# YufengJin/BundleSDF

Hardware: AMD Instinct MI355X
Metric: NeRF training rays/sec + ms/iter, 64-frame pool, 2048 rays/frame (higher is better)
Workload: dtype fp16 table+MLP (MFMA) / fp32 accumulate+Adam (amp)

## Files before the change

bundlesdf_amd/csrc/field_step.hip:

```cpp
#include <algorithm>
#include <cstdlib>
#include <cstring>
#include <array>
#include <type_traits>
#include <vector>

#include "nof_device.h"
#include "ray_trace.h"
#include "mlp_lds.h"

#pragma clang fp contract(off)

#ifndef NOF_ABLATE
#define NOF_ABLATE 0
#endif
#define ABL(bits) (NOF_ABLATE && (a.ablate & (bits)))
#define ABL_HOST(d, bits) (NOF_ABLATE && ((d)->ablate & (bits)))
#define ABL_SKIPQ(q) ((q) < 2 ? (1 << (23 + (q))) : (1 << (27 + (q))))

namespace nof {

typedef _Float16 h8v __attribute__((ext_vector_type(8)));
typedef float f16v __attribute__((ext_vector_type(16)));

// ... 346 lines not shown

__device__ __forceinline__ void corner_rows(const LevelInfo &li, const uint32_t pg[3], uint32_t rows[8]) {
    const uint32_t rs = li.res + 1;
    if (level_dense(rs, li.hs)) {
        const uint32_t base = dense_base_v(li.off, pg, rs), rs2 = rs * rs;
#pragma unroll
        for (int idx = 0; idx < 8; ++idx)
            rows[idx] = base + (idx & 1) + ((idx >> 1) & 1 ? rs : 0u) + ((idx >> 2) & 1 ? rs2 : 0u);
    } else {
#pragma unroll
        for (int idx = 0; idx < 8; ++idx) {
            uint32_t pl[3];
#pragma unroll
            for (int d = 0; d < 3; ++d) pl[d] = pg[d] + ((idx >> d) & 1);
            rows[idx] = li.off + grid_row<3>(0, false, li.hs, li.res, pl);
        }
    }
}

template <typename TT, bool PAIRED = false>
__device__ __forceinline__ void gather_level(const FieldArgs &a, const LevelInfo &li, const float x01[3], float pos[3],
                                             float e[8][2], uint32_t rows[8]) {
    const TT *tab = reinterpret_cast<const TT *>(a.table);
    uint32_t pg[3];
#pragma unroll
    for (int d = 0; d < 3; ++d) {
        pos[d] = __builtin_fmaf(x01[d], li.scale, 0.5f);
        pg[d] = (uint32_t)floorf(pos[d]);
        pos[d] -= (float)pg[d];
    }
    corner_rows(li, pg, rows);
    const uint32_t rs = li.res + 1;
    if (PAIRED && level_dense(rs, li.hs)) {
#pragma unroll
        for (int idx = 0; idx < 8; idx += 2) {
            const TT *p = tab + (size_t)rows[idx] * 2;
            if constexpr (sizeof(TT) == 4) {
                typedef float f4a __attribute__((ext_vector_type(4), aligned(8)));
                const f4a v = *reinterpret_cast<const f4a *>(p);
                e[idx][0] = v.x; e[idx][1] = v.y; e[idx + 1][0] = v.z; e[idx + 1][1] = v.w;
            } else {
                uint2 v;
                __builtin_memcpy(&v, p, 8);
                const __half2 h0 = __builtin_bit_cast(__half2, v.x), h1 = __builtin_bit_cast(__half2, v.y);
                e[idx][0] = __low2float(h0); e[idx][1] = __high2float(h0);
                e[idx + 1][0] = __low2float(h1); e[idx + 1][1] = __high2float(h1);
            }
        }
    } else {
#pragma unroll
        for (int idx = 0; idx < 8; ++idx) {
            const TT *p = tab + (size_t)rows[idx] * 2;
            if constexpr (sizeof(TT) == 4) {
                const float2 v = *reinterpret_cast<const float2 *>(p);
                e[idx][0] = v.x; e[idx][1] = v.y;
            } else {
                const __half2 v = *reinterpret_cast<const __half2 *>(p);
                e[idx][0] = __low2float(v); e[idx][1] = __high2float(v);
            }
        }
    }
}

template <typename TT>
__device__ __forceinline__ void encode_level(const FieldArgs &a, const LevelInfo &li, const float x01[3], float f[2]) {
    float pos[3], e[8][2];
    uint32_t rows[8];
    gather_level<TT, true>(a, li, x01, pos, e, rows);
    f[0] = 0.f; f[1] = 0.f;
#pragma unroll
    for (int idx = 0; idx < 8; ++idx) {
        float w = 1.f;
#pragma unroll
        for (int d = 0; d < 3; ++d) w *= ((idx >> d) & 1) ? pos[d] : 1 - pos[d];
        f[0] = __builtin_fmaf(w, e[idx][0], f[0]);
        f[1] = __builtin_fmaf(w, e[idx][1], f[1]);
    }
}

template <int CTRL> __device__ __forceinline__ int dpp_i(int v) {
    return __builtin_amdgcn_update_dpp(0, v, CTRL, 0xf, 0xf, true);
}
#define DPP_ROW_SHL(n) (0x100 + (n))
#define DPP_ROW_SHR(n) (0x110 + (n))

constexpr uint32_t SLOT_EMPTY = 0xffffffffu;

__device__ __forceinline__ uint32_t lds_cas(uint32_t *p, uint32_t key) {
    uint32_t e = SLOT_EMPTY;
    __hip_atomic_compare_exchange_strong(p, &e, key, __ATOMIC_RELAXED, __ATOMIC_RELAXED, __HIP_MEMORY_SCOPE_WORKGROUP);
    return e;
}

template <bool F16V> __device__ __forceinline__ uint32_t *slot_key(uint32_t *keys, uint32_t s) {
    return keys + (F16V ? 2 * s : s);
}
__device__ __forceinline__ void lds_add_h2(void *vals, uint32_t s, uint32_t packed) {
    __builtin_amdgcn_ds_atomic_fadd_v2f16(
        (__attribute__((address_space(3))) h2v *)(reinterpret_cast<uint32_t *>(vals) + 2 * s),
        __builtin_bit_cast(h2v, packed));
}
template <bool F16V>
__device__ __forceinline__ void lds_add(void *vals, uint32_t s, float v0, float v1) {
    if constexpr (F16V) {
        lds_add_h2(vals, s, __builtin_bit_cast(uint32_t, h2v{(_Float16)v0, (_Float16)v1}));
    } else {
        float *f = reinterpret_cast<float *>(vals) + 2 * s;
        __hip_atomic_fetch_add(f, v0, __ATOMIC_RELAXED, __HIP_MEMORY_SCOPE_WORKGROUP);
        __hip_atomic_fetch_add(f + 1, v1, __ATOMIC_RELAXED, __HIP_MEMORY_SCOPE_WORKGROUP);
    }
}

template <bool F16V>
__device__ __forceinline__ bool lds_probe(uint32_t *keys, void *vals, uint32_t mask, uint32_t key, float v0, float v1,
                                          float *g32, __half *g16) {
    uint32_t s = key;
#pragma unroll 1
    for (int p = 1; p < 16; ++p) {
        s = (s + 1) & mask;
        const uint32_t old = lds_cas(slot_key<F16V>(keys, s), key);
        if (old == SLOT_EMPTY || old == key) {
            lds_add<F16V>(vals, s, v0, v1);
            return true;
        }
    }
    if (g16) atomic_add_h2(g16 + (size_t)key * 2, v0, v1);
    else { atomic_add_f32(g32 + (size_t)key * 2, v0); atomic_add_f32(g32 + (size_t)key * 2 + 1, v1); }
    return false;
}

__device__ __forceinline__ void gather_level_t16(const FieldArgs &a, const LevelInfo &li, h2v g01, float t[8],
                                                 const uint32_t rows[8]) {
    const __half *tab = reinterpret_cast<const __half *>(a.table);
    const uint32_t rs = li.res + 1;
    if (level_dense(rs, li.hs)) {
#pragma unroll
        for (int idx = 0; idx < 8; idx += 2) {
            uint2 v;
            __builtin_memcpy(&v, tab + (size_t)rows[idx] * 2, 8);
            t[idx] = __builtin_amdgcn_fdot2(__builtin_bit_cast(h2v, v.x), g01, 0.f, false);
            t[idx + 1] = __builtin_amdgcn_fdot2(__builtin_bit_cast(h2v, v.y), g01, 0.f, false);
        }
    } else {
#pragma unroll
        for (int idx = 0; idx < 8; ++idx) {
            const uint32_t v = *reinterpret_cast<const uint32_t *>(tab + (size_t)rows[idx] * 2);
            t[idx] = __builtin_amdgcn_fdot2(__builtin_bit_cast(h2v, v), g01, 0.f, false);
        }
    }
}

template <typename TT, bool F16V>
__device__ __forceinline__ void backward_level(const FieldArgs &a, const LevelInfo &li, bool member, bool active,
                                               uint32_t part, const float x01[3], float g0, float g1, h2v g01,
                                               float gx[3], int lane, uint32_t *keys, void *vals, uint32_t mask,
                                               float *g32, __half *g16, int &n_direct) {
    float pos[3];
    uint32_t pg[3], crow[8];
#pragma unroll
    for (int d = 0; d < 3; ++d) {
        pos[d] = __builtin_fmaf(x01[d], li.scale, 0.5f);
        pg[d] = (uint32_t)pos[d];
        pos[d] = __builtin_amdgcn_fractf(pos[d]);
    }
    corner_rows(li, pg, crow);
    if (active && !a.no_dx) {
        float t[8];
        if constexpr (sizeof(TT) == 2) {
            gather_level_t16(a, li, g01, t, crow);
        } else {
            float e[8][2], pos_unused[3];
            uint32_t rows_unused[8];
            gather_level<TT, true>(a, li, x01, pos_unused, e, rows_unused);
#pragma unroll
            for (int k = 0; k < 8; ++k) t[k] = __builtin_fmaf(g1, e[k][1], g0 * e[k][0]);
        }
        float dx[4], ax[4];
#pragma unroll
        for (int j = 0; j < 4; ++j) {
            dx[j] = t[2 * j + 1] - t[2 * j];
            ax[j] = __builtin_fmaf(pos[0], dx[j], t[2 * j]);
        }
        float dy[2], by[2], ux[2];
#pragma unroll
        for (int z = 0; z < 2; ++z) {
            dy[z] = ax[2 * z + 1] - ax[2 * z];
            by[z] = __builtin_fmaf(pos[1], dy[z], ax[2 * z]);
            ux[z] = __builtin_fmaf(pos[1], dx[2 * z + 1] - dx[2 * z], dx[2 * z]);
        }
        gx[0] = __builtin_fmaf(li.scale, __builtin_fmaf(pos[2], ux[1] - ux[0], ux[0]), gx[0]);
        gx[1] = __builtin_fmaf(li.scale, __builtin_fmaf(pos[2], dy[1] - dy[0], dy[0]), gx[1]);
        gx[2] = __builtin_fmaf(li.scale, by[1] - by[0], gx[2]);
    }
    if ABL(1) return;
    const int key = member ? (int)((1u + (pg[0] | (pg[1] << 10) | (pg[2] << 20))) | (part << 31))
                           : (0x40000000 + lane + 1);
    const bool tail = member && (dpp_i<0x130>(key) != key);
    if (ABL(1 << 27)) {
        n_direct += tail ? 1 : 0;
    }
    const bool s1 = dpp_i<DPP_ROW_SHR(1)>(key) == key, s2 = dpp_i<DPP_ROW_SHR(2)>(key) == key;
    const bool s4 = dpp_i<DPP_ROW_SHR(4)>(key) == key, s8 = dpp_i<DPP_ROW_SHR(8)>(key) == key;
    const bool sb15 = __builtin_amdgcn_update_dpp(0, key, 0x142, 0xa, 0xf, false) == key;
    const bool sb31 = __builtin_amdgcn_update_dpp(0, key, 0x143, 0xc, 0xf, false) == key;
    const bool any1 = __any(s1), any2 = __any(s2);
    const bool any4 = __any(s4), any8 = __any(s8);
    const bool anyb15 = __any(sb15), anyb31 = __any(sb31);
    const float h0 = active ? g0 : 0.f, h1 = active ? g1 : 0.f;
    float wxy[4];
#pragma unroll
    for (int j = 0; j < 4; ++j) wxy[j] = ((j & 1) ? pos[0] : 1 - pos[0]) * ((j & 2) ? pos[1] : 1 - pos[1]);
    const float wz0[2] = {(1 - pos[2]) * h0, pos[2] * h0}, wz1[2] = {(1 - pos[2]) * h1, pos[2] * h1};
    float v0[8], v1[8];
#pragma unroll
    for (int idx = 0; idx < 8; ++idx) {
        v0[idx] = wxy[idx & 3] * wz0[idx >> 2];
        v1[idx] = wxy[idx & 3] * wz1[idx >> 2];
    }
    uint32_t pk[8];
    const bool pscan = F16V && !ABL(4096);
    if (pscan) {
#pragma unroll
        for (int idx = 0; idx < 8; ++idx) pk[idx] = __builtin_bit_cast(uint32_t, h2v{(_Float16)v0[idx], (_Float16)v1[idx]});
#define PFMAC_DPP(I, CTRL) "v_pk_fmac_f16_dpp %" #I ", %" #I ", %8 " CTRL "\n"
#define PSCAN_STEP(SK, CTRL)                                                                                      \
        if (any##SK) {                                                                                            \
            const uint32_t m = s##SK ? 0x3C003C00u : 0u;                                                          \
            asm("s_nop 1\n" PFMAC_DPP(0, CTRL) PFMAC_DPP(1, CTRL) PFMAC_DPP(2, CTRL) PFMAC_DPP(3, CTRL)          \
                PFMAC_DPP(4, CTRL) PFMAC_DPP(5, CTRL) PFMAC_DPP(6, CTRL) PFMAC_DPP(7, CTRL)                      \
                : "+v"(pk[0]), "+v"(pk[1]), "+v"(pk[2]), "+v"(pk[3]), "+v"(pk[4]), "+v"(pk[5]), "+v"(pk[6]),     \
                  "+v"(pk[7])                                                                                     \
                : "v"(m));                                                                                        \
        }
        PSCAN_STEP(1, "row_shr:1 row_mask:0xf bank_mask:0xf bound_ctrl:1")
        PSCAN_STEP(2, "row_shr:2 row_mask:0xf bank_mask:0xf bound_ctrl:1")
        PSCAN_STEP(4, "row_shr:4 row_mask:0xf bank_mask:0xf bound_ctrl:1")
        PSCAN_STEP(8, "row_shr:8 row_mask:0xf bank_mask:0xf bound_ctrl:1")
        PSCAN_STEP(b15, "row_bcast:15 row_mask:0xa bank_mask:0xf")
        PSCAN_STEP(b31, "row_bcast:31 row_mask:0xc bank_mask:0xf")
#undef PFMAC_DPP
#undef PSCAN_STEP
    }
#define FMAC_DPP(I, CTRL) "v_fmac_f32_dpp %" #I ", %" #I ", %16 " CTRL "\n"
#define SCAN_STEP(SK, CTRL)                                                                                       \
    if (!pscan && any##SK) {                                                                                      \
        const float m = s##SK ? 1.f : 0.f;                                                                        \
        asm("s_nop 1\n" FMAC_DPP(0, CTRL) FMAC_DPP(1, CTRL) FMAC_DPP(2, CTRL) FMAC_DPP(3, CTRL)                  \
            FMAC_DPP(4, CTRL) FMAC_DPP(5, CTRL) FMAC_DPP(6, CTRL) FMAC_DPP(7, CTRL) FMAC_DPP(8, CTRL)            \
            FMAC_DPP(9, CTRL) FMAC_DPP(10, CTRL) FMAC_DPP(11, CTRL) FMAC_DPP(12, CTRL) FMAC_DPP(13, CTRL)        \
            FMAC_DPP(14, CTRL) FMAC_DPP(15, CTRL)                                                                \
            : "+v"(v0[0]), "+v"(v0[1]), "+v"(v0[2]), "+v"(v0[3]), "+v"(v0[4]), "+v"(v0[5]), "+v"(v0[6]),         \
              "+v"(v0[7]), "+v"(v1[0]), "+v"(v1[1]), "+v"(v1[2]), "+v"(v1[3]), "+v"(v1[4]), "+v"(v1[5]),         \
              "+v"(v1[6]), "+v"(v1[7])                                                                            \
            : "v"(m));                                                                                            \
    }
    SCAN_STEP(1, "row_shr:1 row_mask:0xf bank_mask:0xf bound_ctrl:1")
    SCAN_STEP(2, "row_shr:2 row_mask:0xf bank_mask:0xf bound_ctrl:1")
    SCAN_STEP(4, "row_shr:4 row_mask:0xf bank_mask:0xf bound_ctrl:1")
    SCAN_STEP(8, "row_shr:8 row_mask:0xf bank_mask:0xf bound_ctrl:1")
    SCAN_STEP(b15, "row_bcast:15 row_mask:0xa bank_mask:0xf")
    SCAN_STEP(b31, "row_bcast:31 row_mask:0xc bank_mask:0xf")
#undef FMAC_DPP
#undef SCAN_STEP
    if (!tail) return;
    if (ABL(1 << 26)) {
        n_direct += (v0[0] + v1[7] == 12345.f || (pscan && pk[3] == 12345u)) ? 1 : 0;
        return;
    }
    if constexpr (F16V) {
        if (!pscan) {
#pragma unroll
            for (int idx = 0; idx < 8; ++idx)
                pk[idx] = __builtin_bit_cast(uint32_t, h2v{(_Float16)v0[idx], (_Float16)v1[idx]});
        }
    }
    uint32_t old[8];
#pragma unroll
    for (int idx = 0; idx < 8; ++idx) old[idx] = lds_cas(slot_key<F16V>(keys, crow[idx] & mask), crow[idx]);
    bool all_ok = true;
#pragma unroll
    for (int idx = 0; idx < 8; ++idx) {
        const bool ok = old[idx] == SLOT_EMPTY || old[idx] == crow[idx];
        all_ok = all_ok && ok;
        if constexpr (F16V) {
            lds_add_h2(vals, crow[idx] & mask, ok ? pk[idx] : 0u);
        } else {
            lds_add<F16V>(vals, crow[idx] & mask, ok ? v0[idx] : 0.f, ok ? v1[idx] : 0.f);
        }
    }
    if (__builtin_expect(__any(!all_ok), 0)) {
#pragma unroll
        for (int idx = 0; idx < 8; ++idx)
            if (!(old[idx] == SLOT_EMPTY || old[idx] == crow[idx])) {
                float u0 = v0[idx], u1 = v1[idx];
                if constexpr (F16V) {
                    const h2v q = __builtin_bit_cast(h2v, pk[idx]);
                    u0 = (float)q[0];
                    u1 = (float)q[1];
                }
                n_direct += lds_probe<F16V>(keys, vals, mask, crow[idx], u0, u1, g32, g16) ? 0 : 1;
            }
    }
}

template <bool F16V, int NJ>
__device__ __forceinline__ int flush_group(uint32_t *keys, void *vals, uint32_t s0, int lane, float *g32, __half *g16,
                                           bool no_hbm) {
    uint32_t k[NJ];
    uint32_t vb[NJ];
    float va[NJ], vc[NJ];
#pragma unroll
    for (int j = 0; j < NJ; ++j) {
        const uint32_t sl = s0 + 64 * j + lane;
        if constexpr (F16V) {
            const uint2 kv = reinterpret_cast<const uint2 *>(keys)[sl];
            k[j] = kv.x;
            vb[j] = kv.y;
        } else {
            k[j] = keys[sl];
            const float2 v = reinterpret_cast<float2 *>(vals)[sl];
            va[j] = v.x; vc[j] = v.y;
        }
    }
#pragma unroll
    for (int j = 0; j < NJ; ++j) {
        const uint32_t sl = s0 + 64 * j + lane;
        if constexpr (F16V) {
            reinterpret_cast<uint2 *>(keys)[sl] = make_uint2(0xffffffffu, 0u);
        } else {
            keys[sl] = 0xffffffffu;
            reinterpret_cast<float2 *>(vals)[sl] = make_float2(0.f, 0.f);
        }
    }
    int n = 0;
#pragma unroll
    for (int j = 0; j < NJ; ++j) {
        n += (int)__popcll(__ballot(k[j] != 0xffffffffu));
        if (k[j] != 0xffffffffu && !no_hbm) {
            if constexpr (F16V) {
                typedef _Float16 h2v __attribute__((ext_vector_type(2)));
                __builtin_amdgcn_global_atomic_fadd_v2f16((__attribute__((address_space(1))) h2v *)(g16 + (size_t)k[j] * 2),
                                                          __builtin_bit_cast(h2v, vb[j]));
            } else if (g16) {
                atomic_add_h2(g16 + (size_t)k[j] * 2, va[j], vc[j]);
            } else {
                atomic_add_f32(g32 + (size_t)k[j] * 2, va[j]);
                atomic_add_f32(g32 + (size_t)k[j] * 2 + 1, vc[j]);
            }
        }
// ... 802 lines not shown
            reinterpret_cast<float2 *>(a.tile_aux + slot * TILE_AUX + min(lane, 2))[1] = d;
        }
        float s0, s1, s2, sf;
        half_sums(h == 0 ? rc[0] : rc[1], s0, s1);
        half_sums(h == 0 ? rc[2] : lf, s2, sf);
        reinterpret_cast<float4 *>(a.rrec + slot * TREC)[2] = make_float4(s0, s1, s2, sf);
        cur = nxt;
        nxt = nn;
    }
}

__global__ __launch_bounds__(256) void k_ray_final(FieldArgs a_) {
    const FieldArgs a = step_args(a_);
    const int r = blockIdx.x * blockDim.x + threadIdx.x;
    const int lane = threadIdx.x & 63, wave = threadIdx.x >> 6;
    float v[10];
#pragma unroll
    for (int k = 0; k < 10; ++k) v[k] = 0.f;
    if (r < a.R) {
        const int ntiles = a.S / 32;
        float wtot = 0.f, nvalid = 0.f, lfs = 0.f, lem = 0.f, lsdf = 0.f, lfsr = 0.f;
        float racc[3] = {0.f, 0.f, 0.f};
        int csig = 0, ccol = 0, crcol = 0, crsig = 0;
#pragma unroll 4
        for (int t = 0; t < ntiles; ++t) {
            const size_t slot = (size_t)r * ntiles + t;
            const float4 *q = reinterpret_cast<const float4 *>(a.rrec + slot * TREC);
            const float4 q0 = q[0], q1 = q[1], q2 = q[2];
            const uint8_t fl = a.tile_bwd[slot];
            wtot += q0.x; nvalid += q0.y; lfs += q0.z; lem += q0.w; lsdf += q1.x;
            const int cnt = __float_as_int(q1.y);
            csig += cnt & TC_SIG; ccol += (cnt >> 1) & 1; crcol += (cnt >> 2) & 1; crsig += (cnt >> 3) & 1;
            if (fl == 1 || fl == 3) {
                racc[0] += q2.x; racc[1] += q2.y; racc[2] += q2.z; lfsr += q2.w;
            }
        }
        const float *cx = a.rctx + (size_t)r * RCTX;
        const float tgt[3] = {cx[3], cx[4], cx[5]};
        const int frame = __float_as_int(cx[23]), rtype = __float_as_int(cx[24]);
        const bool vray = nvalid > 0.f && rtype == 0;
        const float rw = vray ? (frame == 0 ? a.ffw : 1.f) : 0.f;
        float drgb[3], lr = 0.f, rgb[3];
#pragma unroll
        for (int cc = 0; cc < 3; ++cc) {
            rgb[cc] = racc[cc] / (wtot + 1e-10f);
            const float e = rgb[cc] - tgt[cc];
            drgb[cc] = a.rgb_w * 2.f * e * rw * a.inv_3R;
            lr += e * e * rw;
        }
        v[0] = a.rgb_w * lr * a.inv_3R;
        v[1] = lfs * rw;
        v[2] = lem * rw;
        v[3] = lsdf * rw;
        v[4] = nvalid;
        v[5] = lfsr * rw;
        v[6] = (float)csig; v[7] = (float)ccol; v[8] = (float)crcol; v[9] = (float)crsig;
        if (a.dbg_rgb) {
            a.dbg_rgb[r * 3] = rgb[0]; a.dbg_rgb[r * 3 + 1] = rgb[1]; a.dbg_rgb[r * 3 + 2] = rgb[2];
        }
        float4 *ra = reinterpret_cast<float4 *>(a.ray_aux + (size_t)r * RAY_AUX);
        ra[0] = make_float4(drgb[0], drgb[1], drgb[2], wtot);
        ra[1] = make_float4(rw, 0.f, 0.f, 0.f);
        float4 *rg = reinterpret_cast<float4 *>(a.ray_grad + (size_t)r * 12);
        rg[0] = make_float4(0.f, 0.f, 0.f, 0.f);
        rg[1] = make_float4(0.f, 0.f, 0.f, 0.f);
        rg[2] = make_float4(0.f, 0.f, 0.f, 0.f);
    }
    __shared__ float s_v[4][10];
#pragma unroll
    for (int k = 0; k < 10; ++k) {
        const float t = wave_sum(v[k]);
        if (lane == 0) s_v[wave][k] = t;
    }
    __syncthreads();
    if (threadIdx.x < 10) {
        const int k = threadIdx.x;
        const float t = s_v[0][k] + s_v[1][k] + s_v[2][k] + s_v[3][k];
        constexpr int slot[10] = {0, 1, 2, 3, 4, 10, 6, 7, 8, 9};
        if (t != 0.f && (k != 5 || a.fs_rgb_w > 0.f)) atomic_add_f32(loss_row(a, (int)blockIdx.x) + slot[k], t);
    }
}

constexpr int ENCODE_GROUP_SMALL = 2;

constexpr int COMPACT_PER_BLOCK = 4096;
__global__ __launch_bounds__(256) void k_compact(const uint8_t *__restrict__ flags, int n, int *__restrict__ list,
                                                 int *__restrict__ count, int per_block, int *__restrict__ clist) {
    __shared__ int s_wave[3][4];
    __shared__ int s_base[3];
    const int lane = threadIdx.x & 63, wave = threadIdx.x >> 6;
    const int fpt = per_block >> 8;
    const int b0 = blockIdx.x * per_block + threadIdx.x * fpt;
    uint8_t fl[16];
    if (fpt == 16 && b0 + 16 <= n) {
        const uint4 v = *reinterpret_cast<const uint4 *>(flags + b0);
        const uint32_t w[4] = {v.x, v.y, v.z, v.w};
#pragma unroll
        for (int k = 0; k < 16; ++k) fl[k] = (uint8_t)(w[k >> 2] >> (8 * (k & 3)));
    } else {
#pragma unroll
        for (int k = 0; k < 16; ++k) fl[k] = (k < fpt && b0 + k < n) ? flags[b0 + k] : 0;
    }
    int mine[3] = {0, 0, 0};
#pragma unroll
    for (int k = 0; k < 16; ++k) {
        mine[0] += fl[k] == 1;
        mine[1] += fl[k] == 2;
        mine[2] += (fl[k] == 1 || fl[k] == 3);
    }
    int pm[3] = {mine[0], mine[1], mine[2]};
#pragma unroll
    for (int o = 1; o < 64; o <<= 1) {
#pragma unroll
        for (int q = 0; q < 3; ++q) {
            const int u = __shfl_up(pm[q], o, 64);
            if (lane >= o) pm[q] += u;
        }
    }
    if (lane == 63) {
#pragma unroll
        for (int q = 0; q < 3; ++q) s_wave[q][wave] = pm[q];
    }
    __syncthreads();
    if (threadIdx.x < 3) {
        const int q = threadIdx.x;
        const int tot = s_wave[q][0] + s_wave[q][1] + s_wave[q][2] + s_wave[q][3];
        int *cnt = count + (q == 0 ? 0 : (q == 1 ? 2 : 1));
        s_base[q] = (tot && (q < 2 || clist)) ? atomicAdd(cnt, tot) : 0;
    }
    __syncthreads();
    int off[3];
#pragma unroll
    for (int q = 0; q < 3; ++q) {
        off[q] = s_base[q] + pm[q] - mine[q];
        for (int w = 0; w < wave; ++w) off[q] += s_wave[q][w];
    }
#pragma unroll
    for (int k = 0; k < 16; ++k) {
        const int i = b0 + k;
        if (fl[k] == 1) list[off[0]++] = i << 5;
        if (fl[k] == 2) list[n - 1 - off[1]++] = (i << 5) | (int)0x80000000;
        if (clist && (fl[k] == 1 || fl[k] == 3)) clist[off[2]++] = i << 5;
    }
}

__device__ __forceinline__ int bwd_entry(const FieldArgs &a, int li, int n_c, int cap) {
    return a.tile_sid[li < n_c ? li : cap - 1 - (li - n_c)];
}

#include "field_mlp_bwd.h"

__device__ __forceinline__ void loss_fold(const float *__restrict__ part, float *__restrict__ loss_acc, int k);

__host__ __device__ constexpr uint32_t scatter_wave_words(uint32_t mask, int VW) {
    return (1 + VW) * (mask + 1) + 160;
}
template <typename TM, typename TT, bool F16V, int WAVES>
__global__ __launch_bounds__(256) __attribute__((amdgpu_num_sgpr(80), amdgpu_waves_per_eu(WAVES, 8))) void k_scatter(FieldArgs a_) {
    const FieldArgs a = step_args(a_);
    extern __shared__ __attribute__((aligned(16))) char smem[];
    const int lane = threadIdx.x & 63;
    const int wave = __builtin_amdgcn_readfirstlane((int)(threadIdx.x >> 6));
    if (blockIdx.x == 0 && wave == 0) loss_fold(a.loss_part, a.loss_acc, lane);
    const int bx = (a.xcd_order & 2) ? xcd_block(blockIdx.x, gridDim.x) : (int)blockIdx.x;
    const int lpw = a.scatter_lpw, ngrp = ((int)a.L + lpw - 1) / lpw;
    const int gw = __builtin_amdgcn_readfirstlane(bx * 4 + wave);
    const int r = __builtin_amdgcn_readfirstlane(gw / ngrp);
    if (r >= a.R || ABL(65536)) return;
    const int lv0 = __builtin_amdgcn_readfirstlane((gw - r * ngrp) * lpw);
    const int nlev = min(lpw, (int)a.L - lv0);
    const int ntiles = a.S / 32;
    const uint8_t *flags = a.tile_bwd + (size_t)r * ntiles;
    const uint8_t fl = lane < ntiles ? flags[lane] : (uint8_t)0;
    uint32_t gm = lane < ntiles ? a.tile_gmask[(size_t)r * ntiles + lane] : 0u;
    const bool tf = fl == 1 || fl == 2;
    if (!__any(tf) || ABL(131072)) return;
    gm = tf ? gm : 0u;
    const uint32_t mask = a.slot_mask;
    constexpr int VW = F16V ? 1 : 2;
    uint32_t *keys = reinterpret_cast<uint32_t *>(smem) + (size_t)wave * scatter_wave_words(mask, VW);
    uint32_t *vals = F16V ? keys + 1 : keys + mask + 1;
    uint16_t *slist = reinterpret_cast<uint16_t *>(keys + (1 + VW) * (mask + 1));
    if constexpr (F16V) {
        for (uint32_t s = lane; s <= mask; s += 64) reinterpret_cast<uint2 *>(keys)[s] = make_uint2(0xffffffffu, 0u);
    } else {
        for (uint32_t s = lane; s <= mask; s += 64) keys[s] = 0xffffffffu;
        for (uint32_t s = lane; s < VW * (mask + 1); s += 64) vals[s] = 0u;
    }
    if ABL(262144) return;
    float *g32 = (sizeof(TM) == 2) ? nullptr : a.grad_table;
    __half *g16 = (sizeof(TM) == 2) ? a.grad_table16 : nullptr;
    const RayCtx c = load_ray(a, r);
    int n_act = 0;
    for (int ch = 0; ch * 64 < a.S; ++ch) {
        const int s = 64 * ch + lane;
        const uint32_t m0 = (uint32_t)__builtin_amdgcn_readlane((int)gm, 2 * ch);
        const uint32_t m1 = 2 * ch + 1 < 64 ? (uint32_t)__builtin_amdgcn_readlane((int)gm, 2 * ch + 1) : 0u;
        const bool cand = s < a.S && (((lane < 32 ? m0 : m1) >> (s & 31)) & 1u);
        const uint64_t b = __ballot(cand);
        if (cand) slist[n_act + (int)__popcll(b & ((1ull << lane) - 1ull))] = (uint16_t)s;
        n_act += (int)__popcll(b);
    }
    n_act = __builtin_amdgcn_readfirstlane(n_act);
    if (n_act == 0) return;
    __builtin_amdgcn_fence(__ATOMIC_SEQ_CST, "wavefront");
    const int nch = (n_act + 63) / 64;
    float sgz[3] = {0.f, 0.f, 0.f}, sg[3] = {0.f, 0.f, 0.f};
    int n_flush = 0, n_direct = 0;
    if (!ABL(32)) {
        typedef typename std::conditional<sizeof(TM) == 2, uint32_t, float2>::type GPair;
        const size_t RS = (size_t)a.R * a.S;
        const int n_it = nlev * nch;
        auto issue = [&](int lv, int ch, float &z, GPair &g, uint32_t &prt) {
            const int j = 64 * ch + lane;
            const int sj_raw = (int)slist[j];
            const int sj = j < n_act ? sj_raw : 0;
            const size_t sid = (size_t)r * a.S + sj;
            prt = sj >= a.N_oct ? 1u : 0u;
            z = a.zbuf[sid];
            g = reinterpret_cast<const GPair *>(a.dfeat)[(size_t)lv * RS + sid];
        };
        float z_nx = 0.f;
        GPair g_nx{};
        uint32_t prt_nx = 0u;
        issue(lv0, 0, z_nx, g_nx, prt_nx);
        int lv = lv0, ch = 0, lv_n = lv0, ch_n = 0;
        for (int it = 0; it < n_it; ++it) {
            const float z = z_nx;
            const GPair gq = g_nx;
            const uint32_t part = prt_nx;
            if (++ch_n == nch) { ch_n = 0; ++lv_n; }
            issue(min(lv_n, (int)a.L - 1), ch_n, z_nx, g_nx, prt_nx);
            const bool member = 64 * ch + lane < n_act;
            float p[3], x[3], g0, g1;
            h2v g01;
            sample_point(load_ray<true>(a, r), z, p, x);
            if constexpr (sizeof(TM) == 2) {
                g01 = __builtin_bit_cast(h2v, gq);
                g0 = (float)g01[0];
                g1 = (float)g01[1];
            } else {
                g01 = h2v{(_Float16)0.f, (_Float16)0.f};
                g0 = gq.x;
                g1 = gq.y;
            }
            const bool act = member && (g0 != 0.f || g1 != 0.f);
            if (ABL(1 << 25)) {
                n_flush += __any(act) ? (int)__popcll(__ballot(act)) : 0;
                n_direct += (__any(act) && lane == 0) ? 64 : 0;
            }
            const bool skipq = ABL(ABL_SKIPQ(lv >> 2));
            if (__any(act) && !skipq) {
                const LevelInfo li = level_info_uniform(a, lv);
                const float x01[3] = {(x[0] + 1) / 2, (x[1] + 1) / 2, (x[2] + 1) / 2};
                float gx[3] = {0.f, 0.f, 0.f};
                backward_level<TT, F16V>(a, li, member, act, part, x01, g0, g1, g01, gx, lane, keys, vals, mask, g32, g16,
                                         n_direct);
#pragma unroll
                for (int i = 0; i < 3; ++i) {
                    sgz[i] = __builtin_fmaf(gx[i], z, sgz[i]);
                    sg[i] += gx[i];
                }
            }
            if (ch == nch - 1 && !ABL(1) && !ABL(1 << 22) && !skipq) {
                const int nfl = flush_table<F16V>(keys, vals, mask, lane, g32, g16, ABL(128));
                n_flush += nfl;
            }
            if (++ch == nch) { ch = 0; ++lv; }
        }
    }
    if (!a.no_dx) {
        float tz[3], t1[3];
#pragma unroll
        for (int i = 0; i < 3; ++i) {
            tz[i] = 0.5f * wave_sum(sgz[i]);
            t1[i] = 0.5f * wave_sum(sg[i]);
        }
        if (lane < 12) {
            const int i = lane >> 2, j = lane & 3;
            const float gzi = i == 0 ? tz[0] : (i == 1 ? tz[1] : tz[2]);
            const float g1i = i == 0 ? t1[0] : (i == 1 ? t1[1] : t1[2]);
            const float dj = j == 0 ? c.dir[0] : (j == 1 ? c.dir[1] : c.dir[2]);
            const float v = j < 3 ? gzi * dj : g1i;
            if (ngrp == 1) a.ray_grad[(size_t)r * 12 + lane] += v;
            else atomic_add_f32(a.ray_grad + (size_t)r * 12 + lane, v);
        }
    }
    if (!a.count_atomics || ABL(16384)) return;
    const float nf = (float)__builtin_amdgcn_readfirstlane(n_flush), nd = wave_sum((float)n_direct);
    float *cnt = a.loss_acc + 8 + 2 * (r & 63);
    if (lane == 0 && nf != 0.f) atomic_add_f32(cnt, nf);
    if (lane == 0 && nd != 0.f) atomic_add_f32(cnt + 1, nd);
}

struct QueryArgs {
    const float *pts;
    const float *gx, *gy, *gz;
    int nx, ny, nz;
    int64_t n;
    const uint8_t *occ;
    int occ_n;
    float *sdf;
};

template <typename TM, typename TT>
__global__ __launch_bounds__(256) void k_query_sdf(FieldArgs a, QueryArgs q) {
    extern __shared__ __attribute__((aligned(16))) char smem[];
    TM *s_fr = reinterpret_cast<TM *>(smem);
    float *s_b = reinterpret_cast<float *>(smem + N_FRAGS * 64 * 8 * sizeof(TM));
    {
        const uint4 *src = reinterpret_cast<const uint4 *>(a.frags);
        uint4 *dst = reinterpret_cast<uint4 *>(s_fr);
        for (int i = threadIdx.x; i < N_FRAGS * 64 * 8 * (int)sizeof(TM) / 16; i += blockDim.x) dst[i] = src[i];
        for (int i = threadIdx.x; i < 5 * 64; i += blockDim.x) s_b[i] = a.bias[i];
    }
    __syncthreads();
    const int lane = threadIdx.x & 63, n = lane & 31, h = lane >> 5;
    const int wave = __builtin_amdgcn_readfirstlane((int)(threadIdx.x >> 6));
    const int64_t ntile = (q.n + 31) / 32;
    for (int64_t t = (int64_t)blockIdx.x * 4 + wave; t < ntile; t += (int64_t)gridDim.x * 4) {
        const int64_t idx = t * 32 + n;
        const bool inb = idx < q.n;
        float x[3] = {0.f, 0.f, 0.f};
        if (inb) {
            if (q.pts) {
#pragma unroll
                for (int d = 0; d < 3; ++d) x[d] = q.pts[idx * 3 + d];
            } else {
                const int64_t k = idx % q.nz, ij = idx / q.nz;
                const int64_t j = ij % q.ny, i = ij / q.ny;
                x[0] = q.gx[i]; x[1] = q.gy[j]; x[2] = q.gz[k];
            }
        }
        bool valid = inb;
        if (inb && q.occ) {
            const float N = (float)q.occ_n;
            uint32_t c[3];
            bool inside = true;
#pragma unroll
            for (int d = 0; d < 3; ++d) {
                inside = inside && fabsf(x[d]) <= 1.f;
                const float f = floorf((x[d] + 1.f) * 0.5f * N);
                c[d] = (uint32_t)fminf(fmaxf(f, 0.f), N - 1.f);
            }
            valid = inside && q.occ[((size_t)c[2] * q.occ_n + c[1]) * q.occ_n + c[0]] != 0;
        }
        if (!__any(valid)) {
            if (inb && h == 0) q.sdf[idx] = 1.f;
            continue;
        }
#pragma unroll
        for (int d = 0; d < 3; ++d) x[d] = fminf(fmaxf(x[d], -1.f), 1.f);
        const float x01[3] = {(x[0] + 1) / 2, (x[1] + 1) / 2, (x[2] + 1) / 2};
        Acts<TM> A;
#pragma unroll
        for (int ss = 0; ss < 2; ++ss) {
#pragma unroll
            for (int qq = 0; qq < 4; ++qq) {
                const int lv = lane_level(ss, qq, h);
                float v[2] = {0.f, 0.f};
                if (inb && lv < (int)a.L) encode_level<TT>(a, level_info(a, lv), x01, v);
                frag_set<TM>(A.X[ss], 2 * qq, v[0]);
                frag_set<TM>(A.X[ss], 2 * qq + 1, v[1]);
            }
        }
        float sdf;
        f16v l2;
        mlp_sdf_net<TM>(LdsW<TM>{s_fr}, s_b, A, lane, sdf, l2);
        if (inb && h == 0) q.sdf[idx] = valid ? sdf : 1.f;
    }
}

#include "field_query.h"
#include "field_render.h"

__device__ __forceinline__ void loss_fold(const float *__restrict__ part, float *__restrict__ loss_acc, int k) {
    if (k >= LOSS_FOLD_N) return;
    constexpr int dst[LOSS_FOLD_N] = {0, 1, 2, 3, 4, 5, LOSS_ACC_COUNTERS, LOSS_ACC_COUNTERS + 1, LOSS_ACC_COUNTERS + 2,
                                      LOSS_ACC_COUNTERS + 3, LOSS_ACC_COUNTERS + 4, LOSS_ACC_COUNTERS + 5,
                                      LOSS_ACC_COUNTERS + 6};
    float s = 0.f;
    for (int c = 0; c < LOSS_COPIES; ++c) s += part[c * LOSS_SLOTS + k];
    loss_acc[dst[k]] += s;
}

__global__ __launch_bounds__(256) void k_quad_mirror(FieldArgs a) {
    __shared__ uint32_t s_off[16], s_rs[16], s_end[16];
    if (threadIdx.x < a.L) {
        const LevelInfo li = level_info(a, threadIdx.x);
        s_off[threadIdx.x] = li.off;
        s_rs[threadIdx.x] = li.res + 1;
        s_end[threadIdx.x] = level_dense(li.res + 1, li.hs) ? li.off + li.hs : 0u;
    }
    __syncthreads();
    uint32_t end = 0;
    for (int l = 0; l < (int)a.L && s_end[l]; ++l) end = s_end[l];
    const uint32_t *t = reinterpret_cast<const uint32_t *>(a.table);
    uint4 *quads = const_cast<uint4 *>(a.quads);
    int lv = 0;
    for (uint32_t i = blockIdx.x * 256u + threadIdx.x; i < end; i += gridDim.x * 256u) {
        while (lv + 1 < (int)a.L && s_off[lv + 1] <= i) ++lv;
        const uint32_t rs = s_rs[lv], hi = i + rs + 1;
        if (hi >= s_end[lv]) continue;
        quads[i] = make_uint4(t[i], t[i + 1], t[i + rs], t[hi]);
    }
}

__global__ void k_zero_i32(int *__restrict__ p, int n) {
    const int i = blockIdx.x * blockDim.x + threadIdx.x;
// ... 610 lines not shown
```

Baseline: 29.21 million.

## Depth-sort scatter sample list by merging two partitions to coalesce grid keys

Measured after the change: 29.08 million. Within noise of the previous version (-0.4%).

```diff
diff --git a/bundlesdf_amd/csrc/field_step.hip b/bundlesdf_amd/csrc/field_step.hip
--- a/bundlesdf_amd/csrc/field_step.hip
+++ b/bundlesdf_amd/csrc/field_step.hip
@@ -522,9 +522,9 @@
 
 template <typename TT, bool F16V>
 __device__ __forceinline__ void backward_level(const FieldArgs &a, const LevelInfo &li, bool member, bool active,
-                                               uint32_t part, const float x01[3], float g0, float g1, h2v g01,
-                                               float gx[3], int lane, uint32_t *keys, void *vals, uint32_t mask,
-                                               float *g32, __half *g16, int &n_direct) {
+                                               const float x01[3], float g0, float g1, h2v g01, float gx[3], int lane,
+                                               uint32_t *keys, void *vals, uint32_t mask, float *g32, __half *g16,
+                                               int &n_direct) {
     float pos[3];
     uint32_t pg[3], crow[8];
 #pragma unroll
@@ -563,8 +563,7 @@
         gx[2] = __builtin_fmaf(li.scale, by[1] - by[0], gx[2]);
     }
     if ABL(1) return;
-    const int key = member ? (int)((1u + (pg[0] | (pg[1] << 10) | (pg[2] << 20))) | (part << 31))
-                           : (0x40000000 + lane + 1);
+    const int key = member ? (int)(1u + (pg[0] | (pg[1] << 10) | (pg[2] << 20))) : (0x40000000 + lane + 1);
     const bool tail = member && (dpp_i<0x130>(key) != key);
     if (ABL(1 << 27)) {
         n_direct += tail ? 1 : 0;
@@ -1673,8 +1672,12 @@
 
 __device__ __forceinline__ void loss_fold(const float *__restrict__ part, float *__restrict__ loss_acc, int k);
 
+constexpr int SCATTER_MAX_S = 320;
+__host__ __device__ constexpr uint32_t scatter_table_words(uint32_t mask, int VW) {
+    return (1 + VW) * (mask + 1) > (uint32_t)SCATTER_MAX_S ? (1 + VW) * (mask + 1) : (uint32_t)SCATTER_MAX_S;
+}
 __host__ __device__ constexpr uint32_t scatter_wave_words(uint32_t mask, int VW) {
-    return (1 + VW) * (mask + 1) + 160;
+    return scatter_table_words(mask, VW) + SCATTER_MAX_S / 2;
 }
 template <typename TM, typename TT, bool F16V, int WAVES>
 __global__ __launch_bounds__(256) __attribute__((amdgpu_num_sgpr(80), amdgpu_waves_per_eu(WAVES, 8))) void k_scatter(FieldArgs a_) {
@@ -1701,7 +1704,63 @@
     constexpr int VW = F16V ? 1 : 2;
     uint32_t *keys = reinterpret_cast<uint32_t *>(smem) + (size_t)wave * scatter_wave_words(mask, VW);
     uint32_t *vals = F16V ? keys + 1 : keys + mask + 1;
-    uint16_t *slist = reinterpret_cast<uint16_t *>(keys + (1 + VW) * (mask + 1));
+    uint16_t *slist = reinterpret_cast<uint16_t *>(keys + scatter_table_words(mask, VW));
+    float *g32 = (sizeof(TM) == 2) ? nullptr : a.grad_table;
+    __half *g16 = (sizeof(TM) == 2) ? a.grad_table16 : nullptr;
+    const RayCtx c = load_ray(a, r);
+    float *zl = reinterpret_cast<float *>(keys);
+    auto candidates = [&](int ch, int s, bool &p1, uint64_t &b0, uint64_t &b1) {
+        const uint32_t m0 = (uint32_t)__builtin_amdgcn_readlane((int)gm, 2 * ch);
+        const uint32_t m1 = 2 * ch + 1 < 64 ? (uint32_t)__builtin_amdgcn_readlane((int)gm, 2 * ch + 1) : 0u;
+        const bool cand = s < a.S && (((lane < 32 ? m0 : m1) >> (s & 31)) & 1u);
+        p1 = s >= a.N_oct;
+        b1 = __ballot(cand && p1);
+        b0 = __ballot(cand && !p1);
+        return cand;
+    };
+    const uint64_t below = (1ull << lane) - 1ull;
+    int n0 = 0, n1 = 0;
+    for (int ch = 0; ch * 64 < a.S; ++ch) {
+        const int s = 64 * ch + lane;
+        bool p1;
+        uint64_t b0, b1;
+        const bool cand = candidates(ch, s, p1, b0, b1);
+        const float z = a.zbuf[(size_t)r * a.S + min(s, a.S - 1)];
+        const int i = p1 ? n1 + (int)__popcll(b1 & below) : n0 + (int)__popcll(b0 & below);
+        if (cand) zl[p1 ? SCATTER_MAX_S - 1 - i : i] = z;
+        n0 += (int)__popcll(b0);
+        n1 += (int)__popcll(b1);
+    }
+    n0 = __builtin_amdgcn_readfirstlane(n0);
+    n1 = __builtin_amdgcn_readfirstlane(n1);
+    const int n_act = n0 + n1;
+    if (n_act == 0) return;
+    __builtin_amdgcn_fence(__ATOMIC_SEQ_CST, "wavefront");
+    {
+        const int top = 1 << (31 - __builtin_clz(max(n0, n1)));
+        int c0 = 0, c1 = 0;
+        for (int ch = 0; ch * 64 < a.S; ++ch) {
+            const int s = 64 * ch + lane;
+            bool p1;
+            uint64_t b0, b1;
+            const bool cand = candidates(ch, s, p1, b0, b1);
+            if ((b0 | b1) == 0) continue;
+            const int i = p1 ? c1 + (int)__popcll(b1 & below) : c0 + (int)__popcll(b0 & below);
+            const float z = zl[cand ? (p1 ? SCATTER_MAX_S - 1 - i : i) : 0];
+            const int nn = p1 ? n0 : n1;
+            int rank = 0;
+            for (int st = top; st; st >>= 1) {
+                const int t = rank + st;
+                const int k = max(min(t, nn) - 1, 0);
+                const float zo = zl[p1 ? k : SCATTER_MAX_S - 1 - k];
+                rank = (t <= nn && (p1 ? zo <= z : zo < z)) ? t : rank;
+            }
+            if (cand) slist[i + rank] = (uint16_t)s;
+            c0 += (int)__popcll(b0);
+            c1 += (int)__popcll(b1);
+        }
+    }
+    __builtin_amdgcn_fence(__ATOMIC_SEQ_CST, "wavefront");
     if constexpr (F16V) {
         for (uint32_t s = lane; s <= mask; s += 64) reinterpret_cast<uint2 *>(keys)[s] = make_uint2(0xffffffffu, 0u);
     } else {
@@ -1709,21 +1768,6 @@
         for (uint32_t s = lane; s < VW * (mask + 1); s += 64) vals[s] = 0u;
     }
     if ABL(262144) return;
-    float *g32 = (sizeof(TM) == 2) ? nullptr : a.grad_table;
-    __half *g16 = (sizeof(TM) == 2) ? a.grad_table16 : nullptr;
-    const RayCtx c = load_ray(a, r);
-    int n_act = 0;
-    for (int ch = 0; ch * 64 < a.S; ++ch) {
-        const int s = 64 * ch + lane;
-        const uint32_t m0 = (uint32_t)__builtin_amdgcn_readlane((int)gm, 2 * ch);
-        const uint32_t m1 = 2 * ch + 1 < 64 ? (uint32_t)__builtin_amdgcn_readlane((int)gm, 2 * ch + 1) : 0u;
-        const bool cand = s < a.S && (((lane < 32 ? m0 : m1) >> (s & 31)) & 1u);
-        const uint64_t b = __ballot(cand);
-        if (cand) slist[n_act + (int)__popcll(b & ((1ull << lane) - 1ull))] = (uint16_t)s;
-        n_act += (int)__popcll(b);
-    }
-    n_act = __builtin_amdgcn_readfirstlane(n_act);
-    if (n_act == 0) return;
     __builtin_amdgcn_fence(__ATOMIC_SEQ_CST, "wavefront");
     const int nch = (n_act + 63) / 64;
     float sgz[3] = {0.f, 0.f, 0.f}, sg[3] = {0.f, 0.f, 0.f};
@@ -1732,26 +1776,23 @@
         typedef typename std::conditional<sizeof(TM) == 2, uint32_t, float2>::type GPair;
         const size_t RS = (size_t)a.R * a.S;
         const int n_it = nlev * nch;
-        auto issue = [&](int lv, int ch, float &z, GPair &g, uint32_t &prt) {
+        auto issue = [&](int lv, int ch, float &z, GPair &g) {
             const int j = 64 * ch + lane;
             const int sj_raw = (int)slist[j];
             const int sj = j < n_act ? sj_raw : 0;
             const size_t sid = (size_t)r * a.S + sj;
-            prt = sj >= a.N_oct ? 1u : 0u;
             z = a.zbuf[sid];
             g = reinterpret_cast<const GPair *>(a.dfeat)[(size_t)lv * RS + sid];
         };
         float z_nx = 0.f;
         GPair g_nx{};
-        uint32_t prt_nx = 0u;
-        issue(lv0, 0, z_nx, g_nx, prt_nx);
+        issue(lv0, 0, z_nx, g_nx);
         int lv = lv0, ch = 0, lv_n = lv0, ch_n = 0;
         for (int it = 0; it < n_it; ++it) {
             const float z = z_nx;
             const GPair gq = g_nx;
-            const uint32_t part = prt_nx;
             if (++ch_n == nch) { ch_n = 0; ++lv_n; }
-            issue(min(lv_n, (int)a.L - 1), ch_n, z_nx, g_nx, prt_nx);
+            issue(min(lv_n, (int)a.L - 1), ch_n, z_nx, g_nx);
             const bool member = 64 * ch + lane < n_act;
             float p[3], x[3], g0, g1;
             h2v g01;
@@ -1775,7 +1816,7 @@
                 const LevelInfo li = level_info_uniform(a, lv);
                 const float x01[3] = {(x[0] + 1) / 2, (x[1] + 1) / 2, (x[2] + 1) / 2};
                 float gx[3] = {0.f, 0.f, 0.f};
-                backward_level<TT, F16V>(a, li, member, act, part, x01, g0, g1, g01, gx, lane, keys, vals, mask, g32, g16,
+                backward_level<TT, F16V>(a, li, member, act, x01, g0, g1, g01, gx, lane, keys, vals, mask, g32, g16,
                                          n_direct);
 #pragma unroll
                 for (int i = 0; i < 3; ++i) {
```
